# Visual-Behavior/detr-tensorflow

Measured on AMD Instinct MI355X. Metric: images/sec training step, DETR-R50 800x1333 bs=8/GPU, higher is better.
Workload: dtype bf16

## Files before the change

detr-tensorflow_amd/csrc/gemm_f32.hip:

```cpp
#include "gemm_core.h"
#include "gemm_bf16_core.h"
#include "gemm_stream.h"

#include "gemm_kernels.h"
#include "gemm_x3.h"
#include "gemm_ring.h"

namespace detr {

struct ReduceOne : detr_reduce_desc {
    int vec;
    int nblocks;
};

template <int G>
__device__ __forceinline__ void splitk_reduce_body(const float *__restrict__ ws, int splits, long long part_stride,
                                                   int rows, int cols, float *__restrict__ C, long long ldc,
                                                   float alpha, const float *__restrict__ scale, int vec,
                                                   const float *__restrict__ rs_ws, float *__restrict__ rs_out,
                                                   float rs_alpha, const int bid, const int nbid,
                                                   const int ts_bm = 0, const int ts_bn = 0, const int ts_tn = 1) {
    constexpr int OUT = 256 / G;
    __shared__ float4 red[G][OUT];
    if (rs_ws) {
        for (int m = bid * 256 + threadIdx.x; m < rows; m += nbid * 256) {
            float t = 0.0f;
            for (int k = 0; k < splits; ++k) t += rs_ws[(long long)k * rows + m];
            rs_out[m] += rs_alpha * t;
        }
    }
    const int lo = threadIdx.x % OUT, grp = threadIdx.x / OUT;
    if (ts_bm > 0) {
        __shared__ float tr[OUT][5];
        const int upt = (ts_bm * ts_bn) >> 2;
        const long long total = part_stride >> 2;
        for (long long base = (long long)bid * OUT; base < total; base += (long long)nbid * OUT) {
            const long long i = base + lo;
            const bool valid = i < total;
            float4 s = make_float4(0.f, 0.f, 0.f, 0.f);
            if (valid) {
                const float *p = ws + i * 4;
#pragma unroll 4
                for (int k = grp; k < splits; k += G) {
                    const float4 v = *reinterpret_cast<const float4 *>(p + k * part_stride);
                    s.x += v.x; s.y += v.y; s.z += v.z; s.w += v.w;
                }
            }
            red[grp][lo] = s;
            __syncthreads();
            if (grp == 0) {
#pragma unroll
                for (int q = 1; q < G; ++q) {
                    const float4 t = red[q][lo];
                    s.x += t.x; s.y += t.y; s.z += t.z; s.w += t.w;
                }
                tr[lo][0] = s.x; tr[lo][1] = s.y; tr[lo][2] = s.z; tr[lo][3] = s.w;
            }
            __syncthreads();
            if (grp == 0 && valid) {
                const int qb = lo & ~3, t = lo & 3;
                const long long iq = base + qb;
                const int tile = (int)(iq / upt), u = (int)(iq - (long long)tile * upt);
                int row0, col;
                slab_ts_unit(u, ts_bm, ts_bn, row0, col);
                const int row = row0 + (tile / ts_tn) * ts_bm + t;
                col += (tile % ts_tn) * ts_bn;
                if (row < rows && col < cols) {
                    const float4 v = make_float4(tr[qb][t], tr[qb + 1][t], tr[qb + 2][t], tr[qb + 3][t]);
                    float4 sc = make_float4(1.f, 1.f, 1.f, 1.f);
                    if (scale) sc = *reinterpret_cast<const float4 *>(scale + col);
                    float4 *dst = reinterpret_cast<float4 *>(C + (long long)row * ldc + col);
                    float4 o = *dst;
                    o.x += alpha * sc.x * v.x; o.y += alpha * sc.y * v.y; o.z += alpha * sc.z * v.z; o.w += alpha * sc.w * v.w;
                    *dst = o;
                }
            }
        }
    } else if (vec) {
        const int c4n = cols >> 2;
        const long long total = (long long)rows * c4n;
        for (long long base = (long long)bid * OUT; base < total; base += (long long)nbid * OUT) {
            const long long i = base + lo;
            const bool valid = i < total;
            int r = 0, c = 0;
            float4 s = make_float4(0.f, 0.f, 0.f, 0.f);
            if (valid) {
                r = (int)(i / c4n);
                c = (int)(i - (long long)r * c4n) * 4;
                const float *p = ws + (long long)r * cols + c;
#pragma unroll 4
                for (int k = grp; k < splits; k += G) {
                    const float4 v = *reinterpret_cast<const float4 *>(p + k * part_stride);
                    s.x += v.x; s.y += v.y; s.z += v.z; s.w += v.w;
                }
            }
            red[grp][lo] = s;
            __syncthreads();
            if (grp == 0 && valid) {
#pragma unroll
                for (int q = 1; q < G; ++q) {
                    const float4 t = red[q][lo];
                    s.x += t.x; s.y += t.y; s.z += t.z; s.w += t.w;
                }
                float4 sc = make_float4(1.f, 1.f, 1.f, 1.f);
                if (scale) sc = *reinterpret_cast<const float4 *>(scale + c);
                float4 *dst = reinterpret_cast<float4 *>(C + (long long)r * ldc + c);
                float4 o = *dst;
                o.x += alpha * sc.x * s.x; o.y += alpha * sc.y * s.y; o.z += alpha * sc.z * s.z; o.w += alpha * sc.w * s.w;
                *dst = o;
            }
            __syncthreads();
        }
    } else {
        const long long total = (long long)rows * cols;
        for (long long i = bid * (long long)blockDim.x + threadIdx.x; i < total; i += (long long)nbid * blockDim.x) {
            const int r = (int)(i / cols), c = (int)(i - (long long)r * cols);
            float s = 0.f;
            for (int k = 0; k < splits; ++k) s += ws[k * part_stride + i];
            C[(long long)r * ldc + c] += alpha * (scale ? scale[c] : 1.0f) * s;
        }
    }
}

constexpr int REDUCE_MANY = 16;
template <int NMAX> struct ReduceArgs { ReduceOne r[NMAX]; };
template <int G, int NMAX>
__global__ __launch_bounds__(256) void splitk_reduce_kernel(ReduceArgs<NMAX> R) {
    const ReduceOne &r = R.r[NMAX == 1 ? 0 : blockIdx.y];
    if ((int)blockIdx.x >= r.nblocks) return;
    splitk_reduce_body<G>(r.ws, r.splits, r.part_stride, r.rows, r.cols, r.C, r.ldc, r.alpha, r.scale, r.vec, r.rs_ws, r.rs_out,
                          r.rs_alpha, blockIdx.x, r.nblocks, r.ts_bm, r.ts_bn, r.ts_tiles_n);
}

static ReduceOne reduce_plan(const detr_reduce_desc &d, bool &small) {
    ReduceOne r;
    static_cast<detr_reduce_desc &>(r) = d;
    if (r.ts_tiles_n <= 0) r.ts_tiles_n = 1;
    r.vec = (r.cols % 4 == 0) && (r.ldc % 4 == 0) && (r.part_stride % 4 == 0) && aligned16(r.ws) && aligned16(r.C) &&
            (!r.scale || aligned16(r.scale));
    const bool ts = r.ts_bm > 0;
    const bool vec_like = r.vec || ts;
    const long long total = (long long)r.rows * (vec_like ? r.cols / 4 : r.cols);
    small = vec_like && total <= 65536 && r.splits >= 8;
    const long long units = ts ? r.part_stride / 4 : total;
    long long grid = vec_like ? (units + (small ? 15 : 63)) / (small ? 16 : 64) : (units + 255) / 256;
    if (grid > 8192) grid = 8192;
    if (grid < 1) grid = 1;
    r.nblocks = (int)grid;
    return r;
}

template <int NMAX>
static void launch_reduce_list(const ReduceOne *r, int n, bool small, hipStream_t s) {
    ReduceArgs<NMAX> R;
    unsigned rx = 1;
    for (int i = 0; i < NMAX; ++i) {
        R.r[i] = r[i < n ? i : 0];
        if ((unsigned)R.r[i].nblocks > rx) rx = (unsigned)R.r[i].nblocks;
    }
    const dim3 grid(rx, (unsigned)n), block(256);
    if (small) hipLaunchKernelGGL((splitk_reduce_kernel<16, NMAX>), grid, block, 0, s, R);
    else hipLaunchKernelGGL((splitk_reduce_kernel<4, NMAX>), grid, block, 0, s, R);
}

void launch_splitk_reduce(const detr_reduce_desc &d, hipStream_t stream) {
    bool small;
    const ReduceOne r = reduce_plan(d, small);
    launch_reduce_list<1>(&r, 1, small, stream);
}

typedef void (*GemmKernel)(GemmArgs);
typedef void (*GemmGroupKernel)(GemmGroupArgs);

template <class F>
static auto by_layout(bool ak, bool bk) {
    return ak ? (bk ? F::template get<true, true>() : F::template get<true, false>())
              : (bk ? F::template get<false, true>() : F::template get<false, false>());
}

template <int BM, int BN, int WGM, int WGN> struct F32Kernels {
    template <bool AK, bool BKC> static GemmKernel get() { return gemm_f32_kernel<BM, BN, WGM, WGN, AK, BKC>; }
};
template <int BM, int BN, bool DB> struct X3Kernels {
    template <bool AK, bool BKC> static GemmKernel get() {
        if constexpr (BM == 192 && !AK) return nullptr;
        else return gemm_x3_kernel<BM, BN, AK, BKC, DB>;
    }
};
template <int BM, int BN, bool A16, bool B16> struct Bf16Kernels {
    template <bool AK, bool BKC> static GemmKernel get() { return gemm_bf16c_kernel<BM, BN, 2, 2, AK, BKC, A16, B16>; }
};
template <int BM, int BN> struct Bf16K64Kernels {
    template <bool AK, bool BKC> static GemmKernel get() { return gemm_bf16c_k64_kernel<BM, BN, 2, 2, AK, BKC>; }
};
struct GroupF32Kernels {
    template <bool AK, bool BKC> static GemmGroupKernel get() { return gemm_f32_group_kernel<64, 64, 2, 2, AK, BKC>; }
};
struct GroupX3Kernels {
    template <bool AK, bool BKC> static GemmGroupKernel get() { return gemm_x3_group_kernel<64, 64, AK, BKC>; }
};
template <bool A16, bool B16> struct GroupBf16Kernels {
    template <bool AK, bool BKC> static GemmGroupKernel get() { return gemm_bf16c_group_kernel<64, 64, 2, 2, AK, BKC, A16, B16>; }
};

template <int BM, int BN>
static GemmKernel gemm_x3_for(bool ak, bool bk) {
    if constexpr (BM != 192) {
        if (tune(T_X3_DB) == 1) return by_layout<X3Kernels<BM, BN, true>>(ak, bk);
    }
    return by_layout<X3Kernels<BM, BN, false>>(ak, bk);
}

template <int BM, int BN>
static GemmKernel gemm_bf16_for(bool ak, bool bk, bool a16, bool b16, bool k64) {
    if constexpr ((BM == 64 && BN == 64) || (BM == 128 && BN == 128)) {
        if (k64 && a16 && b16) return by_layout<Bf16K64Kernels<BM, BN>>(ak, bk);
    }
    if (a16) return b16 ? by_layout<Bf16Kernels<BM, BN, true, true>>(ak, bk) : by_layout<Bf16Kernels<BM, BN, true, false>>(ak, bk);
    return b16 ? by_layout<Bf16Kernels<BM, BN, false, true>>(ak, bk) : by_layout<Bf16Kernels<BM, BN, false, false>>(ak, bk);
}

static GemmGroupKernel gemm_group_for(bool bf16c, bool split3, bool ak, bool bk, bool a16, bool b16) {
    if (!bf16c) return split3 ? by_layout<GroupX3Kernels>(ak, bk) : by_layout<GroupF32Kernels>(ak, bk);
    if (a16) return b16 ? by_layout<GroupBf16Kernels<true, true>>(ak, bk) : by_layout<GroupBf16Kernels<true, false>>(ak, bk);
    return b16 ? by_layout<GroupBf16Kernels<false, true>>(ak, bk) : by_layout<GroupBf16Kernels<false, false>>(ak, bk);
}

static int launch_gemm_tiles(GemmKernel kernel, int bm, int bn, const GemmArgs &g, int batch, hipStream_t s) {
    DETR_REQUIRE(kernel != nullptr && bm > 0 && bn > 0, "gemm: no kernel for this tile, precision and operand layout");
    GemmArgs a = g;
    a.tiles_m = cdiv(g.M, bm);
    a.tiles_n = cdiv(g.N, bn);
    const dim3 grid((unsigned)(a.tiles_m * a.tiles_n), 1, (unsigned)(batch * g.split_k));
    hipLaunchKernelGGL(kernel, grid, dim3(GEMM_THREADS), 0, s, a);
    return 0;
}

}

using namespace detr;

enum GemmTile {
    TILE_64x64 = 0,
    TILE_128x128 = 1,
    TILE_128x64 = 2,
    TILE_128x32 = 3,
    TILE_WIDE = 4,
    TILE_256x64 = 5,
    TILE_RING_128x256 = 6,
    TILE_RING_256x128 = 7,
    TILE_X3_192x128 = 8
};

struct GemmPlan {
    GemmArgs g;
    int batch, split;
    bool ak, bk, bf16c, partial;
    bool split3;
    bool deep;
    GemmTile tile;
    long long part;
    int ts_bm, ts_bn, ts_tn;
    EpiArgs final_e;
    const detr_gemm_desc *d;
};

struct TileDims { int bm, bn, wgm, wgn; bool slab_ts; };
static TileDims gemm_tile_dims(bool bf16c, GemmTile tile) {
    switch (tile) {
        case TILE_64x64: return {64, 64, 2, 2, true};
        case TILE_128x128: return {128, 128, 2, 2, true};
        case TILE_128x64: return {128, 64, 2, 2, true};
        case TILE_128x32: if (!bf16c) return {128, 32, 4, 1, false}; break;
        case TILE_WIDE: if (bf16c) return {64, 128, 2, 2, true}; return {64, 256, 1, 4, false};
        case TILE_256x64: if (!bf16c) return {256, 64, 4, 1, false}; break;
        case TILE_RING_128x256: if (bf16c) return {128, 256, 2, 2, true}; break;
        case TILE_RING_256x128: if (bf16c) return {256, 128, 2, 2, true}; break;
        case TILE_X3_192x128: if (!bf16c) return {192, 128, 2, 2, true}; break;
    }
    return {0, 0, 0, 0, false};
}
static bool gemm_slab_ts(const detr_gemm_desc *d, int split, int batch, GemmTile tile, int &bm, int &bn) {
    const TileDims t = gemm_tile_dims(d->compute == 1, tile);
    bm = t.bm; bn = t.bn;
    return t.slab_ts && split > 1 && batch == 1 && d->N % 4 == 0 && d->ldc % 4 == 0 && aligned16(d->C) && (!d->scale || aligned16(d->scale)) &&
           tune(T_SLAB_TS) != 2;
}
static bool gemm_ring_wgrad_operands(const detr_gemm_desc *d) {
    return d->compute == 1 && d->a_dtype == 1 && d->b_dtype == 1 && !d->a_kcontig && !d->b_kcontig && !d->rowsum_a && d->M % 8 == 0 &&
           d->N % 8 == 0 && d->lda % 8 == 0 && d->ldb % 8 == 0 && aligned16(d->A) && aligned16(d->B) && tune(T_GEMM_RING) != 2 &&
           tune(T_GEMM_RING) != 3;
}

static bool gemm_split3_shape(const detr_gemm_desc *d) {
    return d->compute == 2 && d->N > 32 && (tune(T_SPLIT3_ALL) == 1 || (d->N >= 128 && d->K >= 256 && d->M >= 128));
}
static GemmTile gemm_pick_tile(const detr_gemm_desc *d, int split, int batch) {
    const bool bf16c = d->compute == 1;
    const int force = tune(T_GEMM_TILE);
    GemmTile tile = TILE_64x64;
    if (bf16c) {
        const long long t128 = (long long)cdiv(d->M, 128) * cdiv(d->N, 128) * batch;
        const bool big_split = (d->N >= 128 && d->K >= 16384) || (d->M >= 512 && d->N >= 512 && d->K >= 4096) ||
                               (d->K >= 4096 && ((d->M >= 256 && d->N >= 2048) || (d->M >= 2048 && d->N >= 256)));
        const bool big_plain = (d->K >= 1024 && t128 >= 512) || (d->K >= 512 && d->N >= 512 && t128 >= 1024) ||
                               (d->K >= 512 && d->N >= 256 && t128 >= 2048);
        const bool small = (split > 1) ? !big_split : !big_plain;
        if (force == 2) tile = TILE_128x64;
        else if (force == 5) tile = TILE_WIDE;
        else if (force == 3 || (force == 0 && small)) tile = TILE_64x64;
        else if (force == 0 && split > 1 && d->M <= 64) tile = TILE_WIDE;
        else tile = TILE_128x128;
        int bm, bn;
        if (tile == TILE_128x128 && gemm_ring_wgrad_operands(d) && gemm_slab_ts(d, split, batch, tile, bm, bn)) {
            const int wt = tune(T_RING_WTILE);
            if (wt == 1 && d->N >= 256) tile = TILE_RING_128x256;
            else if (wt == 2 && d->M >= 256) tile = TILE_RING_256x128;
        }
    } else if (gemm_split3_shape(d)) {
        const long long t128 = (long long)cdiv(d->M, 128) * cdiv(d->N, 128) * batch * split;
        if (force == 1 || (force == 0 && t128 >= x3_t128_threshold())) tile = TILE_128x128;
// ... 273 lines not shown
    return (p.tile == TILE_128x128 || p.tile == TILE_RING_128x256 || p.tile == TILE_RING_256x128) && p.batch == 1 && p.split > 1 &&
           p.g.slab_ts && gemm_ring_wgrad_operands(p.d);
}

enum GemmRoute { ROUTE_TILE = 0, ROUTE_STREAM = 1, ROUTE_RING = 2, ROUTE_RING_F32 = 3, ROUTE_LN = 4, ROUTE_RING_WGRAD = 5 };

static GemmRoute gemm_route(const GemmPlan &p, RingPlan &rp) {
    if (p.d->ln_y) return ROUTE_LN;
    const bool ring_first = tune(T_GEMM_STREAM) != 3 && gemm_ring_eligible(p, rp);
    if (!ring_first && gemm_stream_eligible(p)) return ROUTE_STREAM;
    if (ring_first) return ROUTE_RING;
    if (gemm_ring_f32_eligible(p, rp)) return ROUTE_RING_F32;
    if (gemm_ring_wgrad_eligible(p)) return ROUTE_RING_WGRAD;
    return ROUTE_TILE;
}

static detr_reduce_desc gemm_reduce_desc(const GemmPlan &p) {
    const detr_gemm_desc *d = p.d;
    detr_reduce_desc r = {};
    r.ws = d->workspace; r.splits = p.split; r.part_stride = p.part; r.rows = d->M; r.cols = d->N;
    r.C = d->C; r.ldc = d->ldc; r.alpha = p.final_e.alpha; r.scale = p.final_e.scale;
    r.rs_ws = d->rowsum_a ? d->workspace + (long long)p.split * p.part : nullptr;
    r.rs_out = d->rowsum_a; r.rs_alpha = d->rowsum_alpha;
    r.ts_bm = p.ts_bm; r.ts_bn = p.ts_bn; r.ts_tiles_n = p.ts_tn;
    return r;
}

static GemmKernel gemm_tile_kernel(const GemmPlan &p) {
    const bool ak = p.ak, bk = p.bk;
    if (p.bf16c) {
        const bool a16 = p.g.a16, b16 = p.g.b16;
        switch (p.tile) {
            case TILE_64x64: return gemm_bf16_for<64, 64>(ak, bk, a16, b16, p.deep);
            case TILE_128x128: return gemm_bf16_for<128, 128>(ak, bk, a16, b16, p.deep);
            case TILE_128x64: return gemm_bf16_for<128, 64>(ak, bk, a16, b16, false);
            case TILE_WIDE: return gemm_bf16_for<64, 128>(ak, bk, a16, b16, false);
            default: return nullptr;
        }
    }
    if (p.split3) {
        switch (p.tile) {
            case TILE_64x64: return gemm_x3_for<64, 64>(ak, bk);
            case TILE_128x128: return gemm_x3_for<128, 128>(ak, bk);
            case TILE_128x64: return gemm_x3_for<128, 64>(ak, bk);
            case TILE_X3_192x128: return gemm_x3_for<192, 128>(ak, bk);
            default: return nullptr;
        }
    }
    switch (p.tile) {
        case TILE_64x64: return by_layout<F32Kernels<64, 64, 2, 2>>(ak, bk);
        case TILE_128x128: return by_layout<F32Kernels<128, 128, 2, 2>>(ak, bk);
        case TILE_128x64: return by_layout<F32Kernels<128, 64, 2, 2>>(ak, bk);
        case TILE_128x32: return by_layout<F32Kernels<128, 32, 4, 1>>(ak, bk);
        case TILE_WIDE: return by_layout<F32Kernels<64, 256, 1, 4>>(ak, bk);
        case TILE_256x64: return by_layout<F32Kernels<256, 64, 4, 1>>(ak, bk);
        default: return nullptr;
    }
}

static int gemm_launch(const GemmPlan &p, hipStream_t s) {
    const detr_gemm_desc *d = p.d;
    RingPlan rp;
    switch (gemm_route(p, rp)) {
        case ROUTE_LN: return gemm_ln_launch(p, s);
        case ROUTE_STREAM:
            gemm_stream_launch(p, s);
            DETR_LAUNCH_CHECK("gemm (stream)");
            return 0;
        case ROUTE_RING:
            if (gemm_ring_launch(p.g, p.bk, rp, s)) return -1;
            DETR_LAUNCH_CHECK("gemm (ring)");
            if (d->defer_out) d->defer_out->splits = 0;
            return 0;
        case ROUTE_RING_F32:
            if (gemm_ring_f32_launch(p.g, p.bk, rp, s)) return -1;
            DETR_LAUNCH_CHECK("gemm (ring, fp32)");
            if (d->defer_out) d->defer_out->splits = 0;
            return 0;
        case ROUTE_RING_WGRAD:
            if (gemm_ring_wgrad_launch(p.g, p.ts_bm, p.ts_bn, p.split, s)) return -1;
            break;
        case ROUTE_TILE: {
            DETR_REQUIRE(p.tile != TILE_RING_128x256 && p.tile != TILE_RING_256x128, "gemm: the 128 x 256 / 256 x 128 tiles exist for the ring weight gradient only "
                         "(tile-ordered slabs in a workspace of detr_hip_workspace_bytes_gemm bytes are required)");
            const TileDims t = gemm_tile_dims(p.bf16c, p.tile);
            if (launch_gemm_tiles(gemm_tile_kernel(p), t.bm, t.bn, p.g, p.batch, s)) return -1;
            break;
        }
    }
    DETR_LAUNCH_CHECK("gemm");
    if (d->defer_out) {
        d->defer_out->splits = 0;
        if (p.partial) *d->defer_out = gemm_reduce_desc(p);
        return 0;
    }
    if (p.partial) {
        launch_splitk_reduce(gemm_reduce_desc(p), s);
        DETR_LAUNCH_CHECK("gemm split-k reduce");
    }
    return 0;
}

extern "C" int detr_hip_gemm_family(const detr_gemm_desc *d) {
    GemmPlan p;
    if (gemm_prepare(d, p)) return -1;
    RingPlan rp;
    return gemm_route(p, rp);
}

extern "C" int detr_hip_gemm_f32(const detr_gemm_desc *d, void *stream) {
    GemmPlan p;
    if (gemm_prepare(d, p)) return -1;
    return gemm_launch(p, (hipStream_t)stream);
}

extern "C" int detr_hip_gemm_group_f32(const detr_gemm_desc *descs, int32_t n, void *stream) {
    DETR_REQUIRE(descs != nullptr && n >= 1 && n <= 64, "gemm group: 1..64 descriptors");
    hipStream_t s = (hipStream_t)stream;
    int done = 0;
    while (done < n) {
        const int m = (n - done) < GEMM_MAX_GROUP ? (n - done) : GEMM_MAX_GROUP;
        GemmPlan p[GEMM_MAX_GROUP];
        for (int i = 0; i < m; ++i) {
            DETR_REQUIRE(!descs[done + i].ln_y, "gemm group: the fused LayerNorm (ln_y) exists for single launches only");
            if (gemm_prepare(descs + done + i, p[i])) return -1;
        }
        bool same = m > 1 && tune(T_GEMM_GROUP) != 2;
        for (int i = 0; i < m && same; ++i) {
            RingPlan rp;
            same = p[i].tile == TILE_64x64 && p[i].batch == 1 && p[i].bf16c == p[0].bf16c && p[i].split3 == p[0].split3 && p[i].ak == p[0].ak &&
                   p[i].bk == p[0].bk && p[i].g.a16 == p[0].g.a16 && p[i].g.b16 == p[0].g.b16 && (p[i].split == 1 || p[i].partial) &&
                   gemm_route(p[i], rp) == ROUTE_TILE;
        }
        if (!same) {
            for (int i = 0; i < m; ++i)
                if (gemm_launch(p[i], s)) return -1;
            done += m;
            continue;
        }
        GemmGroupArgs G;
        G.n = m;
        G.work_off[0] = 0;
        for (int i = 0; i < m; ++i) {
            G.g[i] = p[i].g;
            G.g[i].tiles_m = cdiv(p[i].g.M, 64);
            G.g[i].tiles_n = cdiv(p[i].g.N, 64);
            G.work_off[i + 1] = G.work_off[i] + G.g[i].tiles_m * G.g[i].tiles_n * p[i].split;
        }
        for (int i = m; i < GEMM_MAX_GROUP; ++i) { G.g[i] = G.g[0]; G.work_off[i + 1] = G.work_off[m]; }
        const dim3 grid((unsigned)G.work_off[m]);
        hipLaunchKernelGGL(gemm_group_for(p[0].bf16c, p[0].split3, p[0].ak, p[0].bk, p[0].g.a16 != 0, p[0].g.b16 != 0), grid, dim3(GEMM_THREADS), 0, s, G);
        DETR_LAUNCH_CHECK("gemm group");
        ReduceOne r[GEMM_MAX_GROUP];
        bool small[GEMM_MAX_GROUP];
        int nr = 0, nsmall = 0;
        for (int i = 0; i < m; ++i) {
            const detr_gemm_desc *d = p[i].d;
            if (d->defer_out) {
                d->defer_out->splits = 0;
                if (p[i].partial) *d->defer_out = gemm_reduce_desc(p[i]);
            } else if (p[i].partial) {
                r[nr] = reduce_plan(gemm_reduce_desc(p[i]), small[nr]);
                nsmall += small[nr++];
            }
        }
        if (nr > 0 && (nsmall == 0 || nsmall == nr)) {
            launch_reduce_list<GEMM_MAX_GROUP>(r, nr, nsmall > 0, s);
            DETR_LAUNCH_CHECK("gemm group split-k reduce");
        } else if (nr > 0) {
            for (int i = 0; i < nr; ++i) launch_reduce_list<1>(&r[i], 1, small[i], s);
            DETR_LAUNCH_CHECK("gemm group split-k reduce (sequential)");
        }
        done += m;
    }
    return 0;
}



extern "C" int detr_hip_splitk_reduce_many(const detr_reduce_desc *descs, int32_t n, void *stream) {
    DETR_REQUIRE(descs != nullptr && n >= 1, "splitk_reduce_many: bad args");
    hipStream_t s = (hipStream_t)stream;
    for (int pass = 0; pass < 2; ++pass) {
        ReduceOne r[REDUCE_MANY];
        int cnt = 0;
        for (int i = 0; i < n; ++i) {
            const detr_reduce_desc &d = descs[i];
            if (d.splits <= 0) continue;
            DETR_REQUIRE(d.ws && d.C && d.rows > 0 && d.cols > 0, "splitk_reduce_many: entry %d is malformed", i);
            DETR_REQUIRE(d.ts_bm == 0 || ((d.ts_bm == 64 || d.ts_bm == 128 || d.ts_bm == 256) && (d.ts_bn == 64 || d.ts_bn == 128 || d.ts_bn == 256) && d.ts_tiles_n > 0 &&
                                          d.part_stride % ((long long)d.ts_bm * d.ts_bn) == 0),
                         "splitk_reduce_many: entry %d has a malformed tile-ordered slab description", i);
            bool small;
            r[cnt] = reduce_plan(d, small);
            if (small != (pass == 0)) continue;
            if (++cnt == REDUCE_MANY) {
                launch_reduce_list<REDUCE_MANY>(r, cnt, pass == 0, s);
                cnt = 0;
            }
        }
        if (cnt > 0) launch_reduce_list<REDUCE_MANY>(r, cnt, pass == 0, s);
    }
    DETR_LAUNCH_CHECK("splitk_reduce_many");
    return 0;
}
```

detr-tensorflow_amd/detr_tf/_hip.py:

```python
import ctypes
import os
from ctypes import POINTER, Structure, byref, c_float, c_int32, c_int64, c_size_t, c_void_p

import torch

_HERE = os.path.dirname(os.path.abspath(__file__))
LIB_PATH = os.environ.get("DETR_HIP_LIB") or os.path.join(os.path.dirname(_HERE), "lib", "libdetr_hip.so")

f32p = c_void_p


class ReduceDesc(Structure):
    _fields_ = [("ws", c_void_p), ("splits", c_int32), ("part_stride", c_int64), ("rows", c_int32), ("cols", c_int32),
                ("C", c_void_p), ("ldc", c_int64), ("alpha", c_float), ("scale", c_void_p),
                ("rs_ws", c_void_p), ("rs_out", c_void_p), ("rs_alpha", c_float),
                ("ts_bm", c_int32), ("ts_bn", c_int32), ("ts_tiles_n", c_int32)]


class GemmDesc(Structure):
    _fields_ = [("M", c_int32), ("N", c_int32), ("K", c_int32),
                ("A", c_void_p), ("lda", c_int64), ("a_kcontig", c_int32),
                ("B", c_void_p), ("ldb", c_int64), ("b_kcontig", c_int32),
                ("C", c_void_p), ("ldc", c_int64),
                ("batch", c_int32), ("batch_inner", c_int32),
# ... 283 lines not shown
    "detr_hip_overlay": [POINTER(OverlayDesc), c_void_p],
    "detr_hip_track": [POINTER(TrackDesc), c_void_p],
    "detr_hip_track_embed": [POINTER(TrackEmbedDesc), c_void_p],
    "detr_hip_track_motion": [POINTER(TrackMotionDesc), c_void_p],
    "detr_hip_fuse_views": [POINTER(TileMergeDesc), c_void_p, POINTER(ctypes.c_double * FUSE_PARAMS), c_void_p, c_void_p],
}
_SIGNATURES_I64 = {
    "detr_hip_attention_dropmask_words": [c_int32, c_int32, c_int32, c_int32],
    "detr_hip_attention_keymask_words": [c_int32, c_int32],
    "detr_hip_colsum_det_scratch_floats": [c_int64, c_int32],
    "detr_hip_conv1x1_bwd_fused_workspace_floats": [c_int64],
    "detr_hip_workspace_bytes_gemm": [POINTER(GemmDesc)],
    "detr_hip_workspace_bytes_conv3x3": [POINTER(Conv3x3Desc), c_int32],
    "detr_hip_workspace_bytes_stem": [POINTER(StemDesc), c_int32],
    "detr_hip_workspace_bytes_layernorm": [POINTER(LayerNormDesc)],
    "detr_hip_workspace_bytes_conv3x3_dilated": [POINTER(Conv3x3DDesc), c_int32],
    "detr_hip_workspace_bytes_overlay": [POINTER(OverlayDesc)],
    "detr_hip_track_state_bytes": [c_int32],
    "detr_hip_track_embed_state_bytes": [c_int32, c_int32],
    "detr_hip_workspace_bytes_track_embed": [POINTER(TrackEmbedDesc)],
    "detr_hip_track_motion_state_bytes": [c_int32],
    "detr_hip_workspace_bytes_track_motion": [POINTER(TrackMotionDesc)],
}
EXPORTED_SYMBOLS = sorted(list(_SIGNATURES) + list(_SIGNATURES_I64) + ["detr_hip_last_error"])
ABI_VERSION = 9
CRITERION_FLOATS = 8
LAYOUT_STRUCTS = {0: ReduceDesc, 1: GemmDesc, 2: Conv3x3Desc, 3: StemDesc, 4: LayerNormDesc, 5: AttnDesc, 6: SetLossDesc, 7: InputDesc,
                  8: PostprocessDesc, 9: MapMatchDesc, 100: DetectDesc, 200: TileMergeDesc, 300: OverlayDesc, 400: TrackDesc,
                  500: TrackEmbedDesc, 600: TrackMotionDesc, 700: Conv3x3DDesc, 800: CocoMatchDesc}

_lib = None


class KernelProfiler:

    def __init__(self, prealloc=0, f32=False):
        self.f32 = f32
        self.records = []
        self._pool = []
        for _ in range(prealloc):
            ev = torch.cuda.Event(enable_timing=True)
            ev.record()
            self._pool.append(ev)

    def _event(self):
        return self._pool.pop() if self._pool else torch.cuda.Event(enable_timing=True)

    def begin(self):
        ev = self._event()
        ev.record()
        return ev

    def end(self, family, flops, ev0, sig=None, nbytes=0.0):
        ev1 = self._event()
        ev1.record()
        self.records.append((family, flops, ev0, ev1, sig, nbytes))

    def by_shape(self, top=40):
        torch.cuda.synchronize()
        agg = {}
        for fam, flops, e0, e1, sig, _nb in self.records:
            d = agg.setdefault((fam, sig), [0, 0.0, 0.0])
            d[0] += 1
            d[1] += e0.elapsed_time(e1)
            d[2] += flops
        rows = sorted(agg.items(), key=lambda kv: -kv[1][1])[:top]
        return [{"family": k[0], "shape": k[1], "launches": v[0], "ms": round(v[1], 3),
                 "tflops": round(v[2] / (v[1] * 1e-3) / 1e12, 2) if v[1] > 0 else 0.0} for k, v in rows]

    def summary(self):
        torch.cuda.synchronize()
        out = {}
        for fam, flops, e0, e1, _sig, nb in self.records:
            d = out.setdefault(fam, {"launches": 0, "ms": 0.0, "flops": 0.0, "bytes": 0.0, "mixed_s": 0.0})
            d["launches"] += 1
            d["ms"] += e0.elapsed_time(e1)
            d["flops"] += flops
            d["bytes"] += nb
            d["mixed_s"] += max(flops / (157.3e12 if fam.startswith("gemm_f32") or self.f32 else 2.5e15), nb / 8.0e12)
        return out


PROFILER = None
DEFER = None
DEFER_WS = None
_defer_top = 0
_defer_outs = set()
COMPUTE_BF16 = 0
WORKSPACE = None


WS_GENERATION = 0
_WS_RETIRED = []
_DEVICE = None


def ensure_workspace(device, floats=2 * 1024 * 1024):
    global WORKSPACE, _DEVICE, WS_GENERATION
    _DEVICE = torch.device(device)
    if WORKSPACE is None or WORKSPACE.device != _DEVICE or WORKSPACE.numel() < floats:
        if WORKSPACE is not None:
            _WS_RETIRED.append(WORKSPACE)
            WS_GENERATION += 1
        WORKSPACE = torch.empty(floats, dtype=torch.float32, device=device)
    return WORKSPACE


def need_workspace(nbytes):
    if WORKSPACE is not None and nbytes > WORKSPACE.numel() * 4:
        ensure_workspace(WORKSPACE.device, max((int(nbytes) + 3) // 4, WORKSPACE.numel() * 3 // 2))
    return WORKSPACE


def workspace_bytes_held():
    n = WORKSPACE.numel() * 4 if WORKSPACE is not None else 0
    return n + sum(t.numel() * 4 for t in _DEFER_CHUNKS) + sum(t.numel() * 4 for t in _WS_RETIRED)


_WS_NEED = {}


def _ws_query(fn, key, *args):
    v = _WS_NEED.get(key)
    if v is None:
        v = int(getattr(load(), fn)(*args))
        if v < 0:
            raise RuntimeError(f"{fn} rejected the descriptor: {load().detr_hip_last_error().decode()}")
        _WS_NEED[key] = v
    return v


DEFER_LIMIT = int(os.environ.get("DETR_HIP_DEFER_MB", "512")) * 1024 * 1024
DEFER_CHUNK = 64 * 1024 * 1024
_DEFER_CHUNKS = []
_defer_chunk_i = 0


def ensure_defer_workspace(device):
    global _DEVICE
    _DEVICE = torch.device(device)
    if _DEFER_CHUNKS and _DEFER_CHUNKS[0].device != _DEVICE:
        _DEFER_CHUNKS.clear()
    return _DEFER_CHUNKS


def begin_deferred_reduces(device):
    global DEFER, _defer_top, _defer_outs, _defer_chunk_i, _defer_pending
    ensure_defer_workspace(device)
    del _WS_RETIRED[:]
    DEFER, _defer_top, _defer_outs, _defer_chunk_i, _defer_pending = [], 0, set(), 0, 0


AFTER_FLUSH = None


def flush_reduces(end=False):
    global DEFER, _defer_top, _defer_outs, _defer_chunk_i, _defer_pending
    if DEFER is None:
        return
    if DEFER:
        arr = (ReduceDesc * len(DEFER))(*DEFER)
        _check(load().detr_hip_splitk_reduce_many(arr, len(DEFER), _stream()), "detr_hip_splitk_reduce_many")
        if AFTER_FLUSH is not None:
            AFTER_FLUSH()
    _defer_top, _defer_outs, _defer_chunk_i, _defer_pending = 0, set(), 0, 0
    DEFER = None if end else []


def _defer_push(rds):
    rds = [r for r in rds if r is not None and r.splits > 0]
    outs = [r.C for r in rds] + [r.rs_out for r in rds if r.rs_out]
    if len(set(outs)) != len(outs) or any(o in _defer_outs for o in outs):
        flush_reduces()
        for r in rds:
            arr = (ReduceDesc * 1)(r)
            _check(load().detr_hip_splitk_reduce_many(arr, 1, _stream()), "detr_hip_splitk_reduce_many")
        if AFTER_FLUSH is not None:
            AFTER_FLUSH()
        return
    DEFER.extend(rds)
    _defer_outs.update(outs)
    if _defer_pending >= DEFER_LIMIT:
        flush_reduces()


_defer_pending = 0


def _defer_slab(nbytes):
    global _defer_top, _defer_chunk_i, _defer_pending
    nbytes = (int(nbytes) + 255) & ~255
    while True:
        if _defer_chunk_i >= len(_DEFER_CHUNKS):
            _DEFER_CHUNKS.append(torch.empty(max(DEFER_CHUNK, nbytes) // 4, dtype=torch.float32, device=_DEVICE))
        chunk = _DEFER_CHUNKS[_defer_chunk_i]
        if _defer_top + nbytes <= chunk.numel() * 4:
            break
        _defer_chunk_i += 1
        _defer_top = 0
    ptr_ = chunk.data_ptr() + _defer_top
    _defer_top += nbytes
    _defer_pending += nbytes
    return ptr_, nbytes


def load():
    global _lib
    if _lib is not None:
        return _lib
    if not os.path.exists(LIB_PATH):
        raise RuntimeError(f"{LIB_PATH} not found: run `python -c 'import __graft_entry__ as g; g.build()'` "
                           "(or `make -C detr-tensorflow_amd`) first; there is no CPU/eager fallback")
    lib = ctypes.CDLL(LIB_PATH)
    for name, argtypes in _SIGNATURES.items():
        fn = getattr(lib, name)
        fn.argtypes = argtypes
        fn.restype = c_int32
    for name, argtypes in _SIGNATURES_I64.items():
        fn = getattr(lib, name)
        fn.argtypes = argtypes
        fn.restype = c_int64
    lib.detr_hip_last_error.argtypes = []
    lib.detr_hip_last_error.restype = ctypes.c_char_p
    if lib.detr_hip_abi_version() != ABI_VERSION:
        raise RuntimeError(f"{LIB_PATH}: ABI version {lib.detr_hip_abi_version()}, this binding speaks {ABI_VERSION}: rebuild the library")
    check_struct_layouts(lib)
    _lib = lib
    return lib


def struct_layout_mirror(S):
    return [ctypes.sizeof(S)] + [getattr(S, f[0]).offset for f in S._fields_]


def check_struct_layouts(lib):
    for which, S in sorted(LAYOUT_STRUCTS.items()):
        want = struct_layout_mirror(S)
        n = max(lib.detr_hip_struct_layout(which, None, 0), 0)
        buf = (c_int32 * n)()
        lib.detr_hip_struct_layout(which, buf, n)
        got = list(buf)
        if got != want:
            raise RuntimeError(f"ctypes mirror of struct {which} ({S.__name__}) does not match {LIB_PATH}: library {got}, mirror {want}")


def set_tuning(name, value):
    if value is None:
        os.environ.pop(name, None)
    else:
        os.environ[name] = str(value)
    _check(load().detr_hip_reload_tuning(), "detr_hip_reload_tuning")
    _WS_NEED.clear()


def _stream():
    return torch.cuda.current_stream().cuda_stream


def _check(rc, what):
    if rc != 0:
        raise RuntimeError(f"{what} failed ({rc}): {load().detr_hip_last_error().decode()}")


def ptr(t):
    return None if t is None else t.data_ptr()


def _f32(t, name="tensor"):
    if t.dtype != torch.float32 or not t.is_cuda:
        raise TypeError(f"{name}: expected a CUDA float32 tensor, got {t.dtype} on {t.device}")
    return t


def _gemm_desc(M, N, K, A, lda, a_kcontig, B, ldb, b_kcontig, C, ldc, *, alpha=1.0, scale=None, bias=None,
               residual=None, ldr=0, mask=None, ldmask=0, act=0, split_k=1, batch=1, batch_inner=1,
               sA=(0, 0), sB=(0, 0), sC=(0, 0), a_off=0, b_off=0, c_off=0, workspace=None, dropout_p=0.0, dropout_seed=0,
               dropout_step=None, compute=None, rowsum_a=None, rowsum_alpha=1.0, ws_slice=None, maskbits_out=None, ln=None,
               res_sub=None):
    d = GemmDesc()
    d.M, d.N, d.K = M, N, K
    res_rows = M
    if res_sub is not None:
        d.res_sub_h, d.res_sub_w = res_sub
        d.res_sub_ho, d.res_sub_wo = (d.res_sub_h + 1) // 2, (d.res_sub_w + 1) // 2
        res_rows = M // max(1, d.res_sub_h * d.res_sub_w) * d.res_sub_ho * d.res_sub_wo
    if ln is not None:
        d.ln_gamma, d.ln_beta, d.ln_y = ln["gamma"].data_ptr(), ln["beta"].data_ptr(), ln["y"].data_ptr()
        d.ln_mean, d.ln_rstd, d.ln_eps = ln["mean"].data_ptr(), ln["rstd"].data_ptr(), float(ln["eps"])
        if ln.get("y2") is not None:
            d.ln_add, d.ln_add_rows, d.ln_y2 = ln["add"].data_ptr(), ln["add"].shape[0], ln["y2"].data_ptr()
        d.ln_y16 = ptr(ln.get("y16"))
    d.A, d.lda, d.a_kcontig = A.data_ptr() + A.element_size() * a_off, lda, int(a_kcontig)
    is16 = lambda t: 1 if (t is not None and t.dtype == torch.bfloat16) else 0
    d.a_dtype, d.c_dtype, d.r_dtype, d.m_dtype = is16(A), is16(C), is16(residual), is16(mask)
    if mask is not None and mask.dtype == torch.uint8:
        d.m_dtype = 2
    if maskbits_out is not None:
        d.maskbits_out, d.ld_maskbits_out = maskbits_out.data_ptr(), maskbits_out.stride(0)
    d.B, d.ldb, d.b_kcontig = B.data_ptr() + B.element_size() * b_off, ldb, int(b_kcontig)
    d.b_dtype = 1 if B.dtype == torch.bfloat16 else 0
    d.C, d.ldc = C.data_ptr() + C.element_size() * c_off, ldc
    d.batch, d.batch_inner = batch, batch_inner
    d.sA0, d.sA1 = sA
    d.sB0, d.sB1 = sB
    d.sC0, d.sC1 = sC
    d.alpha = alpha
    d.scale, d.bias = ptr(scale), ptr(bias)
    d.residual, d.ldr = ptr(residual), ldr
    d.mask, d.ldmask = ptr(mask), ldmask
    d.act, d.split_k = act, split_k
    d.dropout_p, d.dropout_seed = dropout_p, dropout_seed & 0xFFFFFFFF
    d.dropout_step = ptr(dropout_step)
    d.compute = COMPUTE_BF16 if compute is None else int(compute)
    d.rowsum_a, d.rowsum_alpha = ptr(rowsum_a), rowsum_alpha
    ws_need = 0
    if split_k > 1 and batch == 1 and workspace is None and (WORKSPACE is not None or DEFER is not None):
        ws_need = (_ws_query("detr_hip_workspace_bytes_gemm",
                             ("gemm", M, N, K, int(a_kcontig), int(b_kcontig), split_k, d.compute, d.a_dtype, d.b_dtype, ldc % 4,
                              (d.C or 0) % 16, rowsum_a is not None, scale is not None and (d.scale or 0) % 16), byref(d)) + 255) & ~255
    if workspace is None and WORKSPACE is not None and split_k > 1 and batch == 1 and DEFER is None:
        need_workspace(ws_need * (ws_slice[1] if ws_slice else 1))
    ws = workspace if workspace is not None else WORKSPACE
    if ws is None:
        d.workspace, d.workspace_bytes = None, 0
    elif ws_slice is None:
        d.workspace, d.workspace_bytes = ws.data_ptr(), ws.numel() * 4
    else:
        idx, cnt = ws_slice
# ... 401 lines not shown
```

Measured before the change: 528.8.

## Flatten split-k reduce launches into one packed grid with adaptive threads per unit

```diff
diff --git a/detr-tensorflow_amd/csrc/gemm_f32.hip b/detr-tensorflow_amd/csrc/gemm_f32.hip
--- a/detr-tensorflow_amd/csrc/gemm_f32.hip
+++ b/detr-tensorflow_amd/csrc/gemm_f32.hip
@@ -10,129 +10,174 @@
 
 struct ReduceOne : detr_reduce_desc {
     int vec;
+    int groups;
+    int tpu;
     int nblocks;
 };
-
-template <int G>
-__device__ __forceinline__ void splitk_reduce_body(const float *__restrict__ ws, int splits, long long part_stride,
-                                                   int rows, int cols, float *__restrict__ C, long long ldc,
-                                                   float alpha, const float *__restrict__ scale, int vec,
-                                                   const float *__restrict__ rs_ws, float *__restrict__ rs_out,
-                                                   float rs_alpha, const int bid, const int nbid,
-                                                   const int ts_bm = 0, const int ts_bn = 0, const int ts_tn = 1) {
-    constexpr int OUT = 256 / G;
-    __shared__ float4 red[G][OUT];
-    if (rs_ws) {
-        for (int m = bid * 256 + threadIdx.x; m < rows; m += nbid * 256) {
-            float t = 0.0f;
-            for (int k = 0; k < splits; ++k) t += rs_ws[(long long)k * rows + m];
-            rs_out[m] += rs_alpha * t;
-        }
-    }
-    const int lo = threadIdx.x % OUT, grp = threadIdx.x / OUT;
-    if (ts_bm > 0) {
-        __shared__ float tr[OUT][5];
-        const int upt = (ts_bm * ts_bn) >> 2;
-        const long long total = part_stride >> 2;
-        for (long long base = (long long)bid * OUT; base < total; base += (long long)nbid * OUT) {
+constexpr int REDUCE_LOADS = 16;
+constexpr int REDUCE_LDS_UNITS = 1024;
+constexpr long long REDUCE_FILL = 65536;
+
+__device__ __forceinline__ void add4(float4 &s, const float4 &v) { s.x += v.x; s.y += v.y; s.z += v.z; s.w += v.w; }
+
+template <int G, int T>
+__device__ __forceinline__ float4 reduce_unit(const float *__restrict__ p, const int splits, const long long part_stride, const int t,
+                                              const int lo, float4 *red) {
+    constexpr int A = G / T, U = REDUCE_LOADS / A, OUT = 256 / T;
+    static_assert(A >= 1 && U >= 1 && A * T == G, "reduce_unit: T divides G, G / T <= REDUCE_LOADS");
+    float4 acc[A];
+#pragma unroll
+    for (int a = 0; a < A; ++a) acc[a] = make_float4(0.f, 0.f, 0.f, 0.f);
+    if (p) {
+        const int g0 = t * A;
+        p += g0 * part_stride;
+        int k0 = 0;
+        for (; k0 + G * U <= splits; k0 += G * U) {
+            float4 v[U][A];
+#pragma unroll
+            for (int u = 0; u < U; ++u)
+#pragma unroll
+                for (int a = 0; a < A; ++a) v[u][a] = *reinterpret_cast<const float4 *>(p + (k0 + u * G + a) * part_stride);
+#pragma unroll
+            for (int u = 0; u < U; ++u)
+#pragma unroll
+                for (int a = 0; a < A; ++a) add4(acc[a], v[u][a]);
+        }
+        if (k0 < splits) {
+            float4 v[U][A];
+#pragma unroll
+            for (int u = 0; u < U; ++u)
+#pragma unroll
+                for (int a = 0; a < A; ++a) {
+                    const int k = k0 + u * G + a;
+                    v[u][a] = make_float4(0.f, 0.f, 0.f, 0.f);
+                    if (k + g0 < splits) v[u][a] = *reinterpret_cast<const float4 *>(p + k * part_stride);
+                }
+#pragma unroll
+            for (int u = 0; u < U; ++u)
+#pragma unroll
+                for (int a = 0; a < A; ++a)
+                    if (k0 + u * G + a + g0 < splits) add4(acc[a], v[u][a]);
+        }
+    }
+    float4 s = acc[0];
+#pragma unroll
+    for (int a = 1; a < A; ++a) add4(s, acc[a]);
+    if constexpr (T > 1) {
+#pragma unroll
+        for (int a = 0; a < A; ++a) red[(t * A + a) * OUT + lo] = acc[a];
+        __syncthreads();
+        if (t == 0) {
+#pragma unroll
+            for (int q = A; q < G; ++q) add4(s, red[q * OUT + lo]);
+        }
+        __syncthreads();
+    }
+    return s;
+}
+
+template <int G, int T>
+__device__ __forceinline__ void splitk_reduce_units(const ReduceOne &r, const int bid, float4 *red) {
+    constexpr int OUT = 256 / T;
+    const int lo = threadIdx.x % OUT, t = threadIdx.x / OUT;
+    const long long step = (long long)r.nblocks * OUT;
+    const float alpha = r.alpha;
+    if (r.ts_bm > 0) {
+        const int upt = (r.ts_bm * r.ts_bn) >> 2;
+        const long long total = r.part_stride >> 2;
+        for (long long base = (long long)bid * OUT; base < total; base += step) {
             const long long i = base + lo;
             const bool valid = i < total;
-            float4 s = make_float4(0.f, 0.f, 0.f, 0.f);
-            if (valid) {
-                const float *p = ws + i * 4;
-#pragma unroll 4
-                for (int k = grp; k < splits; k += G) {
-                    const float4 v = *reinterpret_cast<const float4 *>(p + k * part_stride);
-                    s.x += v.x; s.y += v.y; s.z += v.z; s.w += v.w;
+            const float4 s = reduce_unit<G, T>(valid ? r.ws + i * 4 : nullptr, r.splits, r.part_stride, t, lo, red);
+            if (t == 0) {
+                const int q = threadIdx.x & 3;
+                const bool odd = q & 1, hi = q & 2;
+                const float ra = __shfl_xor(odd ? s.x : s.y, 1, 64), rb = __shfl_xor(odd ? s.z : s.w, 1, 64);
+                const float m0 = odd ? ra : s.x, m1 = odd ? s.y : ra, m2 = odd ? rb : s.z, m3 = odd ? s.w : rb;
+                const float rc = __shfl_xor(hi ? m0 : m2, 2, 64), rd = __shfl_xor(hi ? m1 : m3, 2, 64);
+                const float o0 = hi ? rc : m0, o1 = hi ? rd : m1, o2 = hi ? m2 : rc, o3 = hi ? m3 : rd;
+                if (valid) {
+                    const long long iq = i - q;
+                    const int tile = (int)(iq / upt), u = (int)(iq - (long long)tile * upt);
+                    int row0, col;
+                    slab_ts_unit(u, r.ts_bm, r.ts_bn, row0, col);
+                    const int row = row0 + (tile / r.ts_tiles_n) * r.ts_bm + q;
+                    col += (tile % r.ts_tiles_n) * r.ts_bn;
+                    if (row < r.rows && col < r.cols) {
+                        float4 sc = make_float4(1.f, 1.f, 1.f, 1.f);
+                        if (r.scale) sc = *reinterpret_cast<const float4 *>(r.scale + col);
+                        float4 *dst = reinterpret_cast<float4 *>(r.C + (long long)row * r.ldc + col);
+                        float4 o = *dst;
+                        o.x += alpha * sc.x * o0; o.y += alpha * sc.y * o1; o.z += alpha * sc.z * o2; o.w += alpha * sc.w * o3;
+                        *dst = o;
+                    }
                 }
             }
-            red[grp][lo] = s;
-            __syncthreads();
-            if (grp == 0) {
-#pragma unroll
-                for (int q = 1; q < G; ++q) {
-                    const float4 t = red[q][lo];
-                    s.x += t.x; s.y += t.y; s.z += t.z; s.w += t.w;
-                }
-                tr[lo][0] = s.x; tr[lo][1] = s.y; tr[lo][2] = s.z; tr[lo][3] = s.w;
-            }
-            __syncthreads();
-            if (grp == 0 && valid) {
-                const int qb = lo & ~3, t = lo & 3;
-                const long long iq = base + qb;
-                const int tile = (int)(iq / upt), u = (int)(iq - (long long)tile * upt);
-                int row0, col;
-                slab_ts_unit(u, ts_bm, ts_bn, row0, col);
-                const int row = row0 + (tile / ts_tn) * ts_bm + t;
-                col += (tile % ts_tn) * ts_bn;
-                if (row < rows && col < cols) {
-                    const float4 v = make_float4(tr[qb][t], tr[qb + 1][t], tr[qb + 2][t], tr[qb + 3][t]);
-                    float4 sc = make_float4(1.f, 1.f, 1.f, 1.f);
-                    if (scale) sc = *reinterpret_cast<const float4 *>(scale + col);
-                    float4 *dst = reinterpret_cast<float4 *>(C + (long long)row * ldc + col);
-                    float4 o = *dst;
-                    o.x += alpha * sc.x * v.x; o.y += alpha * sc.y * v.y; o.z += alpha * sc.z * v.z; o.w += alpha * sc.w * v.w;
-                    *dst = o;
-                }
-            }
-        }
-    } else if (vec) {
-        const int c4n = cols >> 2;
-        const long long total = (long long)rows * c4n;
-        for (long long base = (long long)bid * OUT; base < total; base += (long long)nbid * OUT) {
+        }
+    } else {
+        const int c4n = r.cols >> 2;
+        const long long total = (long long)r.rows * c4n;
+        for (long long base = (long long)bid * OUT; base < total; base += step) {
             const long long i = base + lo;
             const bool valid = i < total;
-            int r = 0, c = 0;
-            float4 s = make_float4(0.f, 0.f, 0.f, 0.f);
+            int rr = 0, c = 0;
             if (valid) {
-                r = (int)(i / c4n);
-                c = (int)(i - (long long)r * c4n) * 4;
-                const float *p = ws + (long long)r * cols + c;
-#pragma unroll 4
-                for (int k = grp; k < splits; k += G) {
-                    const float4 v = *reinterpret_cast<const float4 *>(p + k * part_stride);
-                    s.x += v.x; s.y += v.y; s.z += v.z; s.w += v.w;
-                }
+                rr = (int)(i / c4n);
+                c = (int)(i - (long long)rr * c4n) * 4;
             }
-            red[grp][lo] = s;
-            __syncthreads();
-            if (grp == 0 && valid) {
-#pragma unroll
-                for (int q = 1; q < G; ++q) {
-                    const float4 t = red[q][lo];
-                    s.x += t.x; s.y += t.y; s.z += t.z; s.w += t.w;
-                }
+            const float4 s = reduce_unit<G, T>(valid ? r.ws + (long long)rr * r.cols + c : nullptr, r.splits, r.part_stride, t, lo, red);
+            if (t == 0 && valid) {
                 float4 sc = make_float4(1.f, 1.f, 1.f, 1.f);
-                if (scale) sc = *reinterpret_cast<const float4 *>(scale + c);
-                float4 *dst = reinterpret_cast<float4 *>(C + (long long)r * ldc + c);
+                if (r.scale) sc = *reinterpret_cast<const float4 *>(r.scale + c);
+                float4 *dst = reinterpret_cast<float4 *>(r.C + (long long)rr * r.ldc + c);
                 float4 o = *dst;
                 o.x += alpha * sc.x * s.x; o.y += alpha * sc.y * s.y; o.z += alpha * sc.z * s.z; o.w += alpha * sc.w * s.w;
                 *dst = o;
             }
-            __syncthreads();
-        }
+        }
+    }
+}
+
+constexpr int REDUCE_MANY = 32;
+template <int NMAX> struct ReduceArgs { ReduceOne r[NMAX]; int first[NMAX + 1]; };
+static_assert(sizeof(ReduceArgs<REDUCE_MANY>) <= 4096, "the reduce list is a kernel argument: 4 KB at most");
+template <int NMAX>
+__global__ __launch_bounds__(256) void splitk_reduce_kernel(ReduceArgs<NMAX> R) {
+    __shared__ float4 red[REDUCE_LDS_UNITS];
+    int e = 0;
+    if (NMAX > 1)
+        while (e + 1 < NMAX && (int)blockIdx.x >= R.first[e + 1]) ++e;
+    const ReduceOne &r = R.r[e];
+    const int bid = (int)blockIdx.x - R.first[e], nbid = r.nblocks;
+    if (r.rs_ws) {
+        for (int m = bid * 256 + threadIdx.x; m < r.rows; m += nbid * 256) {
+            float t = 0.0f;
+#pragma unroll 8
+            for (int k = 0; k < r.splits; ++k) t += r.rs_ws[(long long)k * r.rows + m];
+            r.rs_out[m] += r.rs_alpha * t;
+        }
+    }
+    if (r.ts_bm <= 0 && !r.vec) {
+        const long long total = (long long)r.rows * r.cols;
+        for (long long i = bid * 256LL + threadIdx.x; i < total; i += nbid * 256LL) {
+            const int rr = (int)(i / r.cols), c = (int)(i - (long long)rr * r.cols);
+            float s = 0.f;
+            for (int k = 0; k < r.splits; ++k) s += r.ws[k * r.part_stride + i];
+            r.C[(long long)rr * r.ldc + c] += r.alpha * (r.scale ? r.scale[c] : 1.0f) * s;
+        }
+        return;
+    }
+    if (r.groups == 16) {
+        if (r.tpu == 1) splitk_reduce_units<16, 1>(r, bid, red);
+        else if (r.tpu == 4) splitk_reduce_units<16, 4>(r, bid, red);
+        else splitk_reduce_units<16, 16>(r, bid, red);
     } else {
-        const long long total = (long long)rows * cols;
-        for (long long i = bid * (long long)blockDim.x + threadIdx.x; i < total; i += (long long)nbid * blockDim.x) {
-            const int r = (int)(i / cols), c = (int)(i - (long long)r * cols);
-            float s = 0.f;
-            for (int k = 0; k < splits; ++k) s += ws[k * part_stride + i];
-            C[(long long)r * ldc + c] += alpha * (scale ? scale[c] : 1.0f) * s;
-        }
-    }
-}
-
-constexpr int REDUCE_MANY = 16;
-template <int NMAX> struct ReduceArgs { ReduceOne r[NMAX]; };
-template <int G, int NMAX>
-__global__ __launch_bounds__(256) void splitk_reduce_kernel(ReduceArgs<NMAX> R) {
-    const ReduceOne &r = R.r[NMAX == 1 ? 0 : blockIdx.y];
-    if ((int)blockIdx.x >= r.nblocks) return;
-    splitk_reduce_body<G>(r.ws, r.splits, r.part_stride, r.rows, r.cols, r.C, r.ldc, r.alpha, r.scale, r.vec, r.rs_ws, r.rs_out,
-                          r.rs_alpha, blockIdx.x, r.nblocks, r.ts_bm, r.ts_bn, r.ts_tiles_n);
-}
-
-static ReduceOne reduce_plan(const detr_reduce_desc &d, bool &small) {
+        if (r.tpu == 1) splitk_reduce_units<4, 1>(r, bid, red);
+        else splitk_reduce_units<4, 4>(r, bid, red);
+    }
+}
+
+static ReduceOne reduce_plan(const detr_reduce_desc &d) {
     ReduceOne r;
     static_cast<detr_reduce_desc &>(r) = d;
     if (r.ts_tiles_n <= 0) r.ts_tiles_n = 1;
@@ -141,9 +186,13 @@
     const bool ts = r.ts_bm > 0;
     const bool vec_like = r.vec || ts;
     const long long total = (long long)r.rows * (vec_like ? r.cols / 4 : r.cols);
-    small = vec_like && total <= 65536 && r.splits >= 8;
+    r.groups = (vec_like && total <= 65536 && r.splits >= 8) ? 16 : 4;
     const long long units = ts ? r.part_stride / 4 : total;
-    long long grid = vec_like ? (units + (small ? 15 : 63)) / (small ? 16 : 64) : (units + 255) / 256;
+    r.tpu = 1;
+    if (vec_like)
+        while (r.tpu < r.groups && units * r.tpu < REDUCE_FILL) r.tpu *= 4;
+    const int per_block = 256 / r.tpu;
+    long long grid = (units + per_block - 1) / per_block;
     if (grid > 8192) grid = 8192;
     if (grid < 1) grid = 1;
     r.nblocks = (int)grid;
@@ -151,22 +200,19 @@
 }
 
 template <int NMAX>
-static void launch_reduce_list(const ReduceOne *r, int n, bool small, hipStream_t s) {
+static void launch_reduce_list(const ReduceOne *r, int n, hipStream_t s) {
     ReduceArgs<NMAX> R;
-    unsigned rx = 1;
+    R.first[0] = 0;
     for (int i = 0; i < NMAX; ++i) {
         R.r[i] = r[i < n ? i : 0];
-        if ((unsigned)R.r[i].nblocks > rx) rx = (unsigned)R.r[i].nblocks;
-    }
-    const dim3 grid(rx, (unsigned)n), block(256);
-    if (small) hipLaunchKernelGGL((splitk_reduce_kernel<16, NMAX>), grid, block, 0, s, R);
-    else hipLaunchKernelGGL((splitk_reduce_kernel<4, NMAX>), grid, block, 0, s, R);
+        R.first[i + 1] = R.first[i] + (i < n ? R.r[i].nblocks : 0);
+    }
+    hipLaunchKernelGGL((splitk_reduce_kernel<NMAX>), dim3((unsigned)R.first[NMAX]), dim3(256), 0, s, R);
 }
 
 void launch_splitk_reduce(const detr_reduce_desc &d, hipStream_t stream) {
-    bool small;
-    const ReduceOne r = reduce_plan(d, small);
-    launch_reduce_list<1>(&r, 1, small, stream);
+    const ReduceOne r = reduce_plan(d);
+    launch_reduce_list<1>(&r, 1, stream);
 }
 
 typedef void (*GemmKernel)(GemmArgs);
@@ -746,24 +792,19 @@
         hipLaunchKernelGGL(gemm_group_for(p[0].bf16c, p[0].split3, p[0].ak, p[0].bk, p[0].g.a16 != 0, p[0].g.b16 != 0), grid, dim3(GEMM_THREADS), 0, s, G);
         DETR_LAUNCH_CHECK("gemm group");
         ReduceOne r[GEMM_MAX_GROUP];
-        bool small[GEMM_MAX_GROUP];
-        int nr = 0, nsmall = 0;
+        int nr = 0;
         for (int i = 0; i < m; ++i) {
             const detr_gemm_desc *d = p[i].d;
             if (d->defer_out) {
                 d->defer_out->splits = 0;
                 if (p[i].partial) *d->defer_out = gemm_reduce_desc(p[i]);
             } else if (p[i].partial) {
-                r[nr] = reduce_plan(gemm_reduce_desc(p[i]), small[nr]);
-                nsmall += small[nr++];
+                r[nr++] = reduce_plan(gemm_reduce_desc(p[i]));
             }
         }
-        if (nr > 0 && (nsmall == 0 || nsmall == nr)) {
-            launch_reduce_list<GEMM_MAX_GROUP>(r, nr, nsmall > 0, s);
+        if (nr > 0) {
+            launch_reduce_list<GEMM_MAX_GROUP>(r, nr, s);
             DETR_LAUNCH_CHECK("gemm group split-k reduce");
-        } else if (nr > 0) {
-            for (int i = 0; i < nr; ++i) launch_reduce_list<1>(&r[i], 1, small[i], s);
-            DETR_LAUNCH_CHECK("gemm group split-k reduce (sequential)");
         }
         done += m;
     }
@@ -775,26 +816,25 @@
 extern "C" int detr_hip_splitk_reduce_many(const detr_reduce_desc *descs, int32_t n, void *stream) {
     DETR_REQUIRE(descs != nullptr && n >= 1, "splitk_reduce_many: bad args");
     hipStream_t s = (hipStream_t)stream;
-    for (int pass = 0; pass < 2; ++pass) {
-        ReduceOne r[REDUCE_MANY];
-        int cnt = 0;
-        for (int i = 0; i < n; ++i) {
-            const detr_reduce_desc &d = descs[i];
-            if (d.splits <= 0) continue;
-            DETR_REQUIRE(d.ws && d.C && d.rows > 0 && d.cols > 0, "splitk_reduce_many: entry %d is malformed", i);
-            DETR_REQUIRE(d.ts_bm == 0 || ((d.ts_bm == 64 || d.ts_bm == 128 || d.ts_bm == 256) && (d.ts_bn == 64 || d.ts_bn == 128 || d.ts_bn == 256) && d.ts_tiles_n > 0 &&
-                                          d.part_stride % ((long long)d.ts_bm * d.ts_bn) == 0),
-                         "splitk_reduce_many: entry %d has a malformed tile-ordered slab description", i);
-            bool small;
-            r[cnt] = reduce_plan(d, small);
-            if (small != (pass == 0)) continue;
-            if (++cnt == REDUCE_MANY) {
-                launch_reduce_list<REDUCE_MANY>(r, cnt, pass == 0, s);
-                cnt = 0;
-            }
-        }
-        if (cnt > 0) launch_reduce_list<REDUCE_MANY>(r, cnt, pass == 0, s);
-    }
+    for (int i = 0; i < n; ++i) {
+        const detr_reduce_desc &d = descs[i];
+        if (d.splits <= 0) continue;
+        DETR_REQUIRE(d.ws && d.C && d.rows > 0 && d.cols > 0, "splitk_reduce_many: entry %d is malformed", i);
+        DETR_REQUIRE(d.ts_bm == 0 || ((d.ts_bm == 64 || d.ts_bm == 128 || d.ts_bm == 256) && (d.ts_bn == 64 || d.ts_bn == 128 || d.ts_bn == 256) && d.ts_tiles_n > 0 &&
+                                      d.part_stride % ((long long)d.ts_bm * d.ts_bn) == 0),
+                     "splitk_reduce_many: entry %d has a malformed tile-ordered slab description", i);
+    }
+    ReduceOne r[REDUCE_MANY];
+    int cnt = 0;
+    for (int i = 0; i < n; ++i) {
+        if (descs[i].splits <= 0) continue;
+        r[cnt] = reduce_plan(descs[i]);
+        if (++cnt == REDUCE_MANY) {
+            launch_reduce_list<REDUCE_MANY>(r, cnt, s);
+            cnt = 0;
+        }
+    }
+    if (cnt > 0) launch_reduce_list<REDUCE_MANY>(r, cnt, s);
     DETR_LAUNCH_CHECK("splitk_reduce_many");
     return 0;
 }
diff --git a/detr-tensorflow_amd/detr_tf/_hip.py b/detr-tensorflow_amd/detr_tf/_hip.py
--- a/detr-tensorflow_amd/detr_tf/_hip.py
+++ b/detr-tensorflow_amd/detr_tf/_hip.py
@@ -459,6 +459,17 @@
 
 
 AFTER_FLUSH = None
+REDUCE_LOG = None
+_reduce_calls = 0
+
+
+def _log_reduces(rds, queued):
+    global _reduce_calls
+    for i, r in enumerate(rds):
+        REDUCE_LOG.append({"call": _reduce_calls, "launch": i // 32, "queued": bool(queued), "rows": r.rows, "cols": r.cols, "splits": r.splits,
+                           "part_stride": r.part_stride, "ldc": r.ldc, "ts_bm": r.ts_bm, "ts_bn": r.ts_bn, "ts_tiles_n": r.ts_tiles_n,
+                           "rs": bool(r.rs_ws), "scale": bool(r.scale)})
+    _reduce_calls += 1
 
 
 def flush_reduces(end=False):
@@ -467,6 +478,8 @@
         return
     if DEFER:
         arr = (ReduceDesc * len(DEFER))(*DEFER)
+        if REDUCE_LOG is not None:
+            _log_reduces(DEFER, True)
         _check(load().detr_hip_splitk_reduce_many(arr, len(DEFER), _stream()), "detr_hip_splitk_reduce_many")
         if AFTER_FLUSH is not None:
             AFTER_FLUSH()
@@ -481,6 +494,8 @@
         flush_reduces()
         for r in rds:
             arr = (ReduceDesc * 1)(r)
+            if REDUCE_LOG is not None:
+                _log_reduces([r], False)
             _check(load().detr_hip_splitk_reduce_many(arr, 1, _stream()), "detr_hip_splitk_reduce_many")
         if AFTER_FLUSH is not None:
             AFTER_FLUSH()
```

After: 532.2, median of 6. About the same (+0.6%).
